# ecmwf/anemoi-core

Hardware: AMD Instinct MI355X
Metric: forward nodes*channels/sec on O96 GraphTransformer (higher is better)
Workload: dtype bf16; 1 GPU; AnemoiModelEncProcDec forward, O96 data grid (40320 nodes, 84 vars x 2 steps) -> icosphere res 5 hidden mesh (10242 nodes, 81840 edges), GraphTransformer processor 16 layers x 512 ch x 16 heads, enc 62912 / dec 120960 edges, batch 1; parallelism=single GPU, hip_graph=True, graph_equals_eager=True, graph_segments=1

## Files before the change

### anemoi_core_amd/_lib.py

```python
from __future__ import annotations

import ctypes as C
import os
import threading

ABI_VERSION = 13
LIB_PATH = os.path.join(os.path.dirname(os.path.abspath(__file__)), "lib", "libanemoi_hip.so")

F32, BF16, F16 = 0, 1, 2
ACT_NONE, ACT_GELU = 0, 1
E_INVALID, E_UNSUPPORTED, E_LAUNCH = -1, -2, -3

_p, _i64, _i32, _f = C.c_void_p, C.c_int64, C.c_int32, C.c_float

SIGNATURES = {
    "anemoi_hip_abi_version": ([], C.c_int),
    "anemoi_hip_last_error": ([], C.c_char_p),
    "anemoi_gt_attention_fwd": ([_p, _i64, _p, _i64, _p, _i64, _p, _i64, _p, _p, _p, _i64, _p, _i64, _p, _i32, _i32, _i32, _i32, C.c_int, _p], C.c_int),
    "anemoi_gt_attention_bwd": ([_p, _i64, _p, _i64, _p, _i64, _p, _i64, _p, _i64, _p, _p, _i64, _p, _p, _p, _p, _p,
                                 _p, _i64, _p, _i64, _p, _i64, _p, _i64, _p, _p, _i32, _i32, _i32, _i32, _i32, C.c_int, _p], C.c_int),
    "anemoi_gt_attention_dropout_fwd": ([_p, _i64, _p, _i64, _p, _i64, _p, _i64, _p, _p, _p, _i64, _p, _i64, _p, _i32, _i32, _i32, _i32, _f, C.c_uint64,
                                         C.c_int, _p], C.c_int),
    "anemoi_gt_attention_dropout_bwd": ([_p, _i64, _p, _i64, _p, _i64, _p, _i64, _p, _i64, _p, _p, _i64, _p, _p, _p, _p, _p,
                                         _p, _i64, _p, _i64, _p, _i64, _p, _i64, _p, _p, _i32, _i32, _i32, _i32, _i32, _f, C.c_uint64, C.c_int, _p], C.c_int),
    "anemoi_attention_dropout_mask": ([_p, _i32, _i32, _f, C.c_uint64, _p], C.c_int),
    "anemoi_gt_attention_fused_edge_fwd": ([_p, _i64, _p, _i64, _p, _i64, _p, _i32, _p, _p, _p, _p, _p, _i64, _p, _i64, _p, _i32, _i32, _i32, _i32, C.c_int, _p], C.c_int),
    "anemoi_pack_edge_weights": ([_p, _p, _p, _i32, _i32, _i32, C.c_int, _p], C.c_int),
    "anemoi_pack_edge_features": ([_p, _i64, _p, _i32, _i32, _i32, C.c_int, _p], C.c_int),
    "anemoi_reduce_workspace_bytes": ([_i32], _i64),
    "anemoi_layernorm_bwd": ([_p, _i64, _p, _p, _i64, _p, _i64, _p, _p, _p, _i32, _i32, _f, C.c_int, _p], C.c_int),
    "anemoi_colsum": ([_p, _i64, _p, _p, _i32, _i32, C.c_int, _p], C.c_int),
    "anemoi_gelu_fwd": ([_p, _i64, _p, _i64, _i32, _i32, C.c_int, _p], C.c_int),
    "anemoi_gelu_bwd": ([_p, _i64, _p, _i64, _p, _i64, _i32, _i32, C.c_int, _p], C.c_int),
    "anemoi_cond_layernorm_bwd": ([_p, _i64, _p, _i64, _p, _i64, _p, _i64, _p, _i64, _i32, _i32, _f, C.c_int, _p], C.c_int),
    "anemoi_cond_layernorm_fwd": ([_p, _i64, _p, _i64, _p, _i64, _p, _i64, _i32, _i32, _f, C.c_int, _p], C.c_int),
    "anemoi_assemble_input": ([_p, _i64, _i64, _i32, _i32, _p, _i64, _i32, _p, _i64, _i32, _i32, C.c_int, _p], C.c_int),
    "anemoi_assemble_output": ([_p, _i64, _p, _i64, _p, _p, _i64, _i32, _i32, C.c_int, _p], C.c_int),
    "anemoi_assemble_input_norm": ([_p, C.c_int, _i64, _i64, _i32, _i32, _p, _p, _p, _i64, _i32, _p, _i64, _i32, _i32, C.c_int, _p], C.c_int),
    "anemoi_assemble_output_norm": ([_p, _i64, C.c_int, _p, _i64, _p, _p, _p, _p, _i64, _i32, _i32, C.c_int, _p], C.c_int),
    "anemoi_affine_columns": ([_p, _i64, _p, _i64, _p, _p, _i32, _i32, _i32, C.c_int, _p], C.c_int),
    "anemoi_bound_columns": ([_p, _i64, _i32, _i32, _p, _p, _i32, C.c_int, _p], C.c_int),
    "anemoi_layernorm_fwd": ([_p, _i64, _p, _p, _p, _i64, _p, _i64, _i32, _i32, _f, C.c_int, _p], C.c_int),
    "anemoi_gt_attention_fused_edge_bwd_partial_floats": ([_i32, _i32, _i32], _i64),
    "anemoi_gt_attention_fused_edge_bwd": ([_p, _i64, _p, _i64, _p, _i64, _p, _i32, _p, _p, _i64, _p, _p, _i64, _p, _p, _p, _p, _p,
                                            _p, _i64, _p, _i64, _p, _i64, _p, _p, _p, _p, _p, _p, _p, _p, _i64, _p, _i64,
                                            _i32, _i32, _i32, _i32, _i32, C.c_int, _p], C.c_int),
    "anemoi_linear_wgrad_workspace_bytes": ([_i32, _i32, _i32], _i64),
    "anemoi_linear_wgrad": ([_p, _i64, _p, _i64, _p, _i64, _p, _p, _i32, _i32, _i32, C.c_int, _p], C.c_int),
    "anemoi_linear_splitk_f32": ([_p, _i64, _p, _i64, _p, _i64, _i32, _i32, _i32, _i32, C.c_int, _p], C.c_int),
    "anemoi_linear_stats_fwd": ([_p, _i64, _i32, _p, _i64, _p, _p, _i64, _p, _i64, _p, _i32, _i32, C.c_int, _p], C.c_int),
    "anemoi_linear_lnfold_fwd": ([_p, _i64, _i32, _p, _i64, _p, _p, _p, _i32, _f, C.c_int, _p, _i64, _i32, _i32, C.c_int, _p], C.c_int),
    "anemoi_linear_fwd": ([_p, _i64, _i32, _p, _i64, _i32, _p, _i64, _p, _p, _i64, _p, _p, _i64, _p, _p, _i64, _p, _i64, _i32, _i32, C.c_int, C.c_int, _p], C.c_int),
    "anemoi_linear_fwd_pre": ([_p, _i64, _i32, _p, _i64, _i32, _p, _i64, _p, _p, _i64, _p, _p, _i64, _p, _p, _i64, _p, _i64, _p, _i64, _i32, _i32,
                               C.c_int, C.c_int, _p], C.c_int),
    "anemoi_edge_ln_residual_segment_sum_fwd": ([_p, _i64, _p, _i64, _p, _p, _f, _p, _p, _i64, _p, _i64, _i32, _i32, C.c_int, _p], C.c_int),
    "anemoi_segment_sum_rows": ([_p, _i64, _p, _p, _p, _i64, _i32, _i32, C.c_int, _p], C.c_int),
    "anemoi_gather_add_rows": ([_p, _i64, _p, _i64, _p, _p, _i64, _i32, _i32, C.c_int, _p], C.c_int),
    "anemoi_transpose_pad": ([_p, _i64, _p, _i64, _i32, _i32, _i32, C.c_int, _p], C.c_int),
    "anemoi_glu_fwd": ([_p, _i64, _p, _i64, _i32, _i32, _i32, C.c_int, _p], C.c_int),
    "anemoi_glu_bwd": ([_p, _i64, _p, _i64, _p, _i64, _i32, _i32, _i32, C.c_int, _p], C.c_int),
    "anemoi_gather_rows": ([_p, _i64, _p, _p, _i64, _i32, _i32, C.c_int, _p], C.c_int),
    "anemoi_peer_alloc": ([C.POINTER(_p), _i64, _i32], C.c_int),
    "anemoi_peer_free": ([_p], C.c_int),
    "anemoi_peer_export": ([_p, _p], C.c_int),
    "anemoi_peer_open": ([_p, C.POINTER(_p)], C.c_int),
    "anemoi_peer_close": ([_p], C.c_int),
    "anemoi_gt_chain_rows_per_tile": ([_i32], C.c_int),
    "anemoi_gt_chain2_fwd": ([_p, C.c_int, _p], C.c_int),
    "anemoi_gt_rowchain_fwd": ([_p, C.c_int, _p], C.c_int),
    "anemoi_gt_cluster_chain_fwd": ([_p, C.c_int, _p], C.c_int),
    "anemoi_gt_cluster_chain_workspace_bytes": ([], _i64),
    "anemoi_gnn_edge_chain_fwd": ([_p, _i64, _p, _i64, _p, _p, _i64, _p, _p, _p, _p, _p, _p, _p, _p, _p, _f, _p, _i64, _i32, _i32, C.c_int, _p], C.c_int),
    "anemoi_gnn_mlp_chain_fwd": ([_p, _i64, _i32, _p, _p, _p, _p, _p, _p, _p, _p, _f, _p, _i64, _p, _i64, _i32, _i32, C.c_int, _p], C.c_int),
    "anemoi_gnn_node_chain_segsum_fwd": ([_p, _i64, _p, _i64, _p, _p, _p, _p, _p, _p, _p, _p, _p, _f, _p, _i64, _p, _p, _i32, _p, _i64, _i32, _i32,
                                          C.c_int, _p], C.c_int),
    "anemoi_gnn_node_chain_fwd": ([_p, _i64, _p, _i64, _p, _p, _p, _p, _p, _p, _p, _p, _f, _p, _i64, _p, _p, _i32, _p, _i64, _i32, _i32, C.c_int, _p], C.c_int),
    "anemoi_peer_exchange_rows": ([_p, _i64, _p, _p, _i32, _i32, _i32, _p, _p, _i64, _p], C.c_int),
}


EXPERIMENT_SIGNATURES = {
    "anemoi_gt_chain_fwd": ([_p, C.c_int, _p], C.c_int),
    "anemoi_gnn_edge_chain_timeline": ([_p, _i64, _p, _i64, _p, _p, _i64, _p, _p, _p, _p, _p, _p, _p, _p, _p, _f, _p, _i64, _i32, _p, _p], C.c_int),
}


class HipLibraryError(RuntimeError):
    pass


_lock = threading.Lock()
_lib = None


def load(path: str | None = None):
    global _lib
    if _lib is not None:
        return _lib
    with _lock:
        if _lib is not None:
            return _lib
        path = path or os.environ.get("ANEMOI_HIP_LIB", LIB_PATH)
        if not os.path.exists(path):
            raise HipLibraryError(
                f"{path} not found: build it with `python -m anemoi_core_amd.build` (hipcc, gfx950). "
                "anemoi_core_amd has no CPU / eager fallback."
            )
        try:
            lib = C.CDLL(path)
        except OSError as e:
            raise HipLibraryError(f"cannot load {path}: {e}") from e
        for name, (argtypes, restype) in SIGNATURES.items():
            try:
                fn = getattr(lib, name)
            except AttributeError as e:
                raise HipLibraryError(f"{path} does not export {name}; rebuild the library") from e
            fn.argtypes = argtypes
            fn.restype = restype
        for name, (argtypes, restype) in EXPERIMENT_SIGNATURES.items():
            fn = getattr(lib, name, None)
            if fn is not None:
# ... 18 lines not shown
```

### anemoi_core_amd/build.py

```python
from __future__ import annotations

import os
import shutil
import subprocess
import sys
from concurrent.futures import ThreadPoolExecutor

PKG = os.path.dirname(os.path.abspath(__file__))
REPO = os.path.dirname(PKG)
CSRC = os.path.join(PKG, "csrc")
LIBDIR = os.path.join(PKG, "lib")
LIBPATH = os.path.join(LIBDIR, "libanemoi_hip.so")
EXT_PATH = os.path.join(LIBDIR, "libanemoi_torch.so")
INCLUDE = os.path.join(REPO, "include")

SOURCES = ["lib.cpp", "gt_attention.hip", "gt_attention_bwd.hip", "rowwise.hip", "rowwise_bwd.hip", "linear.hip", "wgrad.hip", "peer.hip", "gt_chain2.hip", "gt_rowchain.hip", "gt_cluster_chain.hip", "gnn_chain.hip"]
EXPERIMENT_SOURCES = ["experiments/gt_chain.hip", "experiments/gnn_chain2.hip"]
EXP_LIBPATH = os.path.join(LIBDIR, "libanemoi_hip_exp.so")
ARCH = "gfx950"


def _hipcc() -> str:
    for cand in (os.environ.get("HIPCC"), shutil.which("hipcc"), "/opt/rocm/bin/hipcc"):
        if cand and os.path.exists(cand):
            return cand
    raise RuntimeError("hipcc not found (need ROCm >= 7.0)")


def _newer(target: str, deps: list[str]) -> bool:
    if not os.path.exists(target):
        return False
    t = os.path.getmtime(target)
    return all(os.path.getmtime(d) <= t for d in deps)


def _deps(path: str, dirs: list[str], seen: set | None = None) -> list[str]:
    import re

    seen = set() if seen is None else seen
    if path in seen:
        return []
    seen.add(path)
    out = [path]
    for inc in re.findall(r'^\s*#include\s+"([^"]+)"', open(path).read(), flags=re.M):
        for d in [os.path.dirname(path), *dirs]:
            cand = os.path.join(d, inc)
            if os.path.exists(cand):
                out += _deps(cand, dirs, seen)
                break
    return out


def build_library(force: bool = False, verbose: bool = True, extra_flags: tuple[str, ...] = (), experiments: bool = False) -> str:
    os.makedirs(LIBDIR, exist_ok=True)
    objdir = os.path.join(LIBDIR, "obj_exp" if experiments else "obj")
    os.makedirs(objdir, exist_ok=True)
    hipcc = _hipcc()
    headers = [os.path.join(CSRC, "common.h"), os.path.join(CSRC, "chain_core.h"), os.path.join(CSRC, "chain2_core.h"), os.path.join(CSRC, "gnn_chain_args.h"), os.path.join(INCLUDE, "anemoi_hip.h")]
    flags = ["-O3", "-std=c++17", "-fPIC", f"--offload-arch={ARCH}", "-I", INCLUDE, "-I", CSRC, "-Wall", "-Wno-unused-function", *extra_flags]
    sources, libpath = SOURCES, LIBPATH
    inc_dirs = [CSRC, INCLUDE] + ([os.path.join(CSRC, "experiments")] if experiments else [])
    if experiments:
        flags += ["-DANEMOI_EXPERIMENTS", "-I", os.path.join(CSRC, "experiments")]
        headers.append(os.path.join(CSRC, "experiments", "anemoi_hip_experiments.h"))
        sources, libpath = SOURCES + EXPERIMENT_SOURCES, EXP_LIBPATH

    def compile_one(src: str) -> str:
        path = os.path.join(CSRC, src)
        obj = os.path.join(objdir, os.path.splitext(os.path.basename(src))[0] + ".o")
        if not force and _newer(obj, _deps(path, inc_dirs)):
            return obj
        cmd = [hipcc, *flags, "-x", "hip", "-c", path, "-o", obj]
        if verbose:
            print("[build]", " ".join(cmd), flush=True)
        subprocess.run(cmd, check=True)
        return obj

    with ThreadPoolExecutor(max_workers=min(4, len(sources))) as ex:
        objs = list(ex.map(compile_one, sources))
    if force or not _newer(libpath, objs):
        cmd = [hipcc, "-shared", "-fPIC", f"--offload-arch={ARCH}", "-o", libpath, *objs]
        if verbose:
            print("[build]", " ".join(cmd), flush=True)
        subprocess.run(cmd, check=True)
    if not experiments:
        build_torch_extension(hipcc, force=force, verbose=verbose)
    return libpath


def build_torch_extension(hipcc: str, force: bool = False, verbose: bool = True) -> str:
    import torch

    src = os.path.join(CSRC, "torch_binding.cpp")
    stamp = EXT_PATH + ".torch_version"
    stamped = open(stamp).read().strip() if os.path.exists(stamp) else None
    if not force and stamped in (None, torch.__version__) and _newer(EXT_PATH, [src, os.path.join(INCLUDE, "anemoi_hip.h"), LIBPATH]):
        if stamped is None:
            open(stamp, "w").write(torch.__version__)
        return EXT_PATH
    troot = os.path.dirname(torch.__file__)
    rocm = os.environ.get("ROCM_PATH", "/opt/rocm")
    cmd = [hipcc, "-O2", "-std=c++17", "-fPIC", "-shared", "-D__HIP_PLATFORM_AMD__=1", "-DUSE_ROCM=1",
           f"-D_GLIBCXX_USE_CXX11_ABI={int(torch._C._GLIBCXX_USE_CXX11_ABI)}", "-I", INCLUDE, "-I", os.path.join(troot, "include"),
           "-I", os.path.join(troot, "include", "torch", "csrc", "api", "include"), "-I", os.path.join(rocm, "include"), src, "-o", EXT_PATH,
           "-L", LIBDIR, "-lanemoi_hip", "-L", os.path.join(troot, "lib"), "-lc10", "-lc10_hip", "-ltorch_cpu", "-ltorch", "-ltorch_hip",
           "-Wl,-rpath,$ORIGIN"]
    if verbose:
        print("[build]", " ".join(cmd), flush=True)
    subprocess.run(cmd, check=True)
    open(stamp, "w").write(torch.__version__)
    return EXT_PATH
# ... 5 lines not shown
```

### anemoi_core_amd/csrc/gt_chain2.hip

```cpp
#include "chain2_core.h"

namespace anemoi {

struct Chain2Args {
  const void* attn;  int64_t ld_attn;
  const void* xres;  int64_t ld_x;
  const char* wp;
  const char* w1;    int hc;
  const char* w2;
  const char* wq;    int qc;
  int qn;
  int q_cols;
  const void* vec;
  float eps1, epsq;
  const void* extra; int64_t ld_extra;
  void* xout;        int64_t ld_out;
  void* qout;        int64_t ld_q;
  int n_rows, rows_per_tile, n_tiles;
  int prio_a;
  int prio_q;
  int dbg;
  int warm;
  int b_delay;
  unsigned long long* timeline;
};
constexpr int kTl2Slots = 48;
constexpr int kRed2Off = 3 * kBufBytes;
constexpr int kVecOff = kRed2Off + kPanel * 4 * 2 * 4;
constexpr int kVecMaxElems = 6144;
constexpr int kChain2Smem = kVecOff + kVecMaxElems * 2;
constexpr int kVecMaxElemsTl = 5120;
constexpr int kTl2Off = kVecOff + kVecMaxElemsTl * 2;
static_assert(kChain2Smem <= 160 * 1024 && kTl2Off + 8 * kTl2Slots * 8 <= 160 * 1024, "LDS budget");

struct Ctx2 {
  int lane, wq, wave;
  uint32_t loff;
  int tl_n;
};
template <bool TL>
__device__ __forceinline__ void stamp2(Ctx2& c, unsigned char* smem) {
  if constexpr (TL) {
    if (c.tl_n < kTl2Slots) {
      const unsigned long long now = __builtin_readcyclecounter();
      if (c.lane == 0) reinterpret_cast<unsigned long long*>(smem + kTl2Off)[c.wave * kTl2Slots + c.tl_n] = now;
    }
    ++c.tl_n;
  }
}
struct VecCopy {
  u32x4 v[2];
  __device__ __forceinline__ void request(const Chain2Args& a, int tid) {
    const int n16 = (1024 + 512 * a.hc + a.q_cols) / 8;
// ... 264 lines not shown
  if (c.wave < 4) {
    if (kExperiments && a.prio_a == 2) __builtin_amdgcn_s_setprio(2);
    role_a<T, TL, PART>(a, c, smem);
  } else {
    role_b<T, TL>(a, c, smem);
  }
  if constexpr (TL) {
    asm volatile("s_waitcnt lgkmcnt(0)" ::: "memory");
    if (c.lane < kTl2Slots)
      a.timeline[((size_t)blockIdx.x * 8 + c.wave) * kTl2Slots + c.lane] =
          c.lane < c.tl_n ? reinterpret_cast<const unsigned long long*>(smem + kTl2Off)[c.wave * kTl2Slots + c.lane] : 0ull;
  }
}

template <typename T>
static int launch_chain2(const Chain2Args& a, hipStream_t st) {
  static PerDeviceOnce attr_once;
  attr_once.run([&] {
    (void)hipFuncSetAttribute(reinterpret_cast<const void*>(&gt_chain2_kernel<T>), hipFuncAttributeMaxDynamicSharedMemorySize, kChain2Smem);
    (void)hipFuncSetAttribute(reinterpret_cast<const void*>(&gt_chain2_kernel<T, false, true>), hipFuncAttributeMaxDynamicSharedMemorySize, kChain2Smem);
  });
  static const int even_grid = ANEMOI_EXPERIMENT_ENV("ANEMOI_CHAIN2_EVEN_GRID", 1, 0, 1);
  int grid = a.n_tiles < 256 ? a.n_tiles : 256;
  static const int max_grid = ANEMOI_EXPERIMENT_ENV("ANEMOI_CHAIN2_MAX_GRID", 256, 8, 256);
  if (even_grid && a.n_tiles > 256) {
    const int rounds = (a.n_tiles + max_grid - 1) / max_grid;
    grid = (a.n_tiles + rounds - 1) / rounds;
  }
#ifdef ANEMOI_EXPERIMENTS
  if (a.timeline != nullptr) {
    static PerDeviceOnce tl_once;
    tl_once.run([&] {
      (void)hipFuncSetAttribute(reinterpret_cast<const void*>(&gt_chain2_kernel<T, true>), hipFuncAttributeMaxDynamicSharedMemorySize, kTl2Off + 8 * kTl2Slots * 8);
      (void)hipFuncSetAttribute(reinterpret_cast<const void*>(&gt_chain2_kernel<T, true, true>), hipFuncAttributeMaxDynamicSharedMemorySize, kTl2Off + 8 * kTl2Slots * 8);
    });
    if (grid < 256) hipLaunchKernelGGL((gt_chain2_kernel<T, true, true>), dim3(grid), dim3(512), kTl2Off + 8 * kTl2Slots * 8, st, a);
    else hipLaunchKernelGGL((gt_chain2_kernel<T, true>), dim3(grid), dim3(512), kTl2Off + 8 * kTl2Slots * 8, st, a);
    return check_launch("gt_chain2_kernel<timeline>");
  }
#endif
  if (grid < 256) hipLaunchKernelGGL((gt_chain2_kernel<T, false, true>), dim3(grid), dim3(512), kChain2Smem, st, a);
  else hipLaunchKernelGGL((gt_chain2_kernel<T>), dim3(grid), dim3(512), kChain2Smem, st, a);
  return check_launch("gt_chain2_kernel");
}

}

using namespace anemoi;

extern "C" int anemoi_gt_chain_rows_per_tile(int32_t n_rows) {
  static const int forced = env_int(getenv("ANEMOI_CHAIN_ROWS"), 0, 0, kPanel);
  (void)n_rows;
  return forced > 0 ? forced : kPanel;
}

extern "C" int anemoi_gt_chain2_fwd(const anemoi_gt_chain2_args_t* p, anemoi_dtype_t dtype, void* stream) {
  ANEMOI_REQUIRE(p != nullptr, "gt_chain2_fwd: null argument block");
  ANEMOI_REQUIRE(dtype == ANEMOI_BF16 || dtype == ANEMOI_F16, "gt_chain2_fwd: 16-bit model dtypes only");
  ANEMOI_REQUIRE(p->n_rows >= 0 && p->channels == kCh, "gt_chain2_fwd: channels=%d (this kernel is built for %d)", p->channels, kCh);
  if (p->n_rows == 0) return ANEMOI_OK;
  const bool narrow = p->q_out_features > 0 && p->q_out_features < kCh;
  ANEMOI_REQUIRE(p->hidden > 0 && p->hidden % kCh == 0 && p->q_out_features >= 0 && (narrow ? p->q_out_features % 128 == 0 : p->q_out_features % kCh == 0),
                 "gt_chain2_fwd: hidden=%d must be a multiple of %d, q_out_features=%d a multiple of %d (or 128, 256, 384)", p->hidden, kCh, p->q_out_features, kCh);
  const int n_vec = 2 * kCh + p->hidden + p->q_out_features;
  if (n_vec > (p->timeline != nullptr ? kVecMaxElemsTl : kVecMaxElems)) return ANEMOI_E_UNSUPPORTED;
  ANEMOI_REQUIRE(p->attn && p->x_res && p->wp && p->w1 && p->w2 && p->vec && (p->x_out || p->q_out_features > 0), "gt_chain2_fwd: null operand");
  ANEMOI_REQUIRE(p->q_out_features == 0 || (p->wq && p->q_out), "gt_chain2_fwd: the trailing projection needs wq and q_out");
  ANEMOI_REQUIRE(p->extra == nullptr || p->x_out != nullptr, "gt_chain2_fwd: a second residual needs x_out");
  const auto al16 = [](const void* q) { return (reinterpret_cast<uintptr_t>(q) & 15) == 0; };
  ANEMOI_REQUIRE(al16(p->attn) && al16(p->x_res) && al16(p->wp) && al16(p->w1) && al16(p->w2) && al16(p->x_out) && al16(p->wq) && al16(p->q_out) &&
                     al16(p->extra) && al16(p->vec),
                 "gt_chain2_fwd: operands must be 16-byte aligned");
  ANEMOI_REQUIRE(p->ld_attn >= kCh && p->ld_x >= kCh && (p->x_out == nullptr || (p->ld_out >= kCh && p->ld_out % 8 == 0)) && p->ld_attn % 8 == 0 && p->ld_x % 8 == 0 &&
                     (p->extra == nullptr || (p->ld_extra >= kCh && p->ld_extra % 8 == 0)) &&
                     (p->q_out_features == 0 || (p->ld_q >= p->q_out_features && p->ld_q % 8 == 0)),
                 "gt_chain2_fwd: leading dimensions too small or not multiples of 8 elements (rows move as 16-byte pieces)");
  Chain2Args a{};
  a.attn = p->attn; a.ld_attn = p->ld_attn;
  a.xres = p->x_res; a.ld_x = p->ld_x;
  a.wp = (const char*)p->wp;
  a.w1 = (const char*)p->w1; a.hc = p->hidden / kCh;
  a.w2 = (const char*)p->w2;
  a.wq = (const char*)p->wq; a.qc = narrow ? 1 : p->q_out_features / kCh;
  a.qn = narrow ? p->q_out_features / 128 : 0; a.q_cols = p->q_out_features;
  a.vec = p->vec;
  a.eps1 = p->ln1_eps; a.epsq = p->lnq_eps;
  a.extra = p->extra; a.ld_extra = p->ld_extra;
  a.xout = p->x_out; a.ld_out = p->ld_out;
  a.qout = p->q_out; a.ld_q = p->ld_q;
  if (!kExperiments && p->timeline != nullptr) {
    set_error("gt_chain2_fwd: the in-kernel timeline is part of the experiments build only (python -m anemoi_core_amd.build --experiments)");
    return ANEMOI_E_UNSUPPORTED;
  }
  a.timeline = reinterpret_cast<unsigned long long*>(p->timeline);
  static const int prio_a = ANEMOI_EXPERIMENT_ENV("ANEMOI_CHAIN2_PRIO_A", 0, 0, 2);
  a.prio_a = prio_a;
  static const int dbg = ANEMOI_EXPERIMENT_ENV("ANEMOI_CHAIN2_DBG", 0, 0, 15);
  a.dbg = dbg;
  static const int prio_q = ANEMOI_EXPERIMENT_ENV("ANEMOI_CHAIN2_PRIO_Q", 0, 0, 1);
  a.prio_q = prio_q;
  static const int warm = ANEMOI_EXPERIMENT_ENV("ANEMOI_CHAIN2_WARM", 1, 0, 1);
  a.warm = warm;
  static const int b_delay = ANEMOI_EXPERIMENT_ENV("ANEMOI_CHAIN2_B_DELAY", 0, 0, 40);
  a.b_delay = b_delay;
  a.n_rows = p->n_rows;
  a.rows_per_tile = p->rows_per_tile > 0 ? p->rows_per_tile : anemoi_gt_chain_rows_per_tile(p->n_rows);
  ANEMOI_REQUIRE(a.rows_per_tile <= kPanel, "gt_chain2_fwd: rows_per_tile=%d exceeds the %d-row panel", a.rows_per_tile, kPanel);
  a.n_tiles = (a.n_rows + a.rows_per_tile - 1) / a.rows_per_tile;
  hipStream_t st = as_stream(stream);
  return dtype == ANEMOI_BF16 ? launch_chain2<bf16_t>(a, st) : launch_chain2<f16_t>(a, st);
}
```

### include/anemoi_hip.h

```cpp
#ifndef ANEMOI_HIP_H
#define ANEMOI_HIP_H

#include <stdint.h>

#ifdef __cplusplus
extern "C" {
#endif

#define ANEMOI_HIP_ABI_VERSION 13

typedef enum { ANEMOI_F32 = 0, ANEMOI_BF16 = 1, ANEMOI_F16 = 2 } anemoi_dtype_t;
typedef enum { ANEMOI_ACT_NONE = 0, ANEMOI_ACT_GELU = 1 } anemoi_act_t;

#define ANEMOI_OK 0
#define ANEMOI_E_INVALID (-1)
#define ANEMOI_E_UNSUPPORTED (-2)
#define ANEMOI_E_LAUNCH (-3)

int anemoi_hip_abi_version(void);
const char* anemoi_hip_last_error(void);

int anemoi_gt_attention_fwd(const void* q, int64_t ldq, const void* k, int64_t ldk, const void* v, int64_t ldv,
                            const void* e, int64_t lde, const int32_t* row, const int32_t* colptr,
                            const void* addend, int64_t ldadd, void* out, int64_t ldo, float* lse,
                            int32_t n_dst, int32_t n_src, int32_t H, int32_t C, anemoi_dtype_t dtype, void* stream);

int anemoi_gt_attention_bwd(const void* q, int64_t ldq, const void* k, int64_t ldk, const void* v, int64_t ldv,
                            const void* e, int64_t lde, const void* out, int64_t ldo, const float* lse,
                            const void* d_out, int64_t lddo, const int32_t* row, const int32_t* colptr,
                            const int32_t* rowptr, const int32_t* edge_ids, const int32_t* edge_dst,
                            void* dq, int64_t lddq, void* dk, int64_t lddk, void* dv, int64_t lddv, void* de, int64_t ldde,
                            float* p_ws, float* ds_ws, int32_t n_dst, int32_t n_src, int32_t n_edges, int32_t H, int32_t C,
                            anemoi_dtype_t dtype, void* stream);

int anemoi_gt_attention_dropout_fwd(const void* q, int64_t ldq, const void* k, int64_t ldk, const void* v, int64_t ldv,
                                    const void* e, int64_t lde, const int32_t* row, const int32_t* colptr,
                                    const void* addend, int64_t ldadd, void* out, int64_t ldo, float* lse,
                                    int32_t n_dst, int32_t n_src, int32_t H, int32_t C, float drop_p, uint64_t drop_seed,
                                    anemoi_dtype_t dtype, void* stream);
int anemoi_gt_attention_dropout_bwd(const void* q, int64_t ldq, const void* k, int64_t ldk, const void* v, int64_t ldv,
                                    const void* e, int64_t lde, const void* out, int64_t ldo, const float* lse,
                                    const void* d_out, int64_t lddo, const int32_t* row, const int32_t* colptr,
                                    const int32_t* rowptr, const int32_t* edge_ids, const int32_t* edge_dst,
                                    void* dq, int64_t lddq, void* dk, int64_t lddk, void* dv, int64_t lddv, void* de, int64_t ldde,
                                    float* p_ws, float* ds_ws, int32_t n_dst, int32_t n_src, int32_t n_edges, int32_t H, int32_t C,
                                    float drop_p, uint64_t drop_seed, anemoi_dtype_t dtype, void* stream);
int anemoi_attention_dropout_mask(float* out, int32_t n_edges, int32_t H, float drop_p, uint64_t drop_seed, void* stream);

int anemoi_gt_attention_fused_edge_fwd(const void* q, int64_t ldq, const void* k, int64_t ldk, const void* v, int64_t ldv,
                                       const float* edge_feat, int32_t fe_pad, const float* w_packed,
                                       const int32_t* row, const int32_t* colptr, const int32_t* dst_order, const void* addend, int64_t ldadd,
                                       void* out, int64_t ldo, float* lse, int32_t n_dst, int32_t n_src, int32_t H,
                                       int32_t C, anemoi_dtype_t dtype, void* stream);

int64_t anemoi_gt_attention_fused_edge_bwd_partial_floats(int32_t H, int32_t C, int32_t fe_pad);
int anemoi_gt_attention_fused_edge_bwd(const void* q, int64_t ldq, const void* k, int64_t ldk, const void* v, int64_t ldv,
                                       const float* edge_feat, int32_t fe_pad, const float* w_packed, const void* out, int64_t ldo,
                                       const float* lse, const void* d_out, int64_t lddo, const int32_t* row, const int32_t* colptr,
                                       const int32_t* rowptr, const int32_t* edge_ids, const int32_t* edge_dst, void* dq,
                                       int64_t lddq, void* dk, int64_t lddk, void* dv, int64_t lddv, float* d_w_packed,
                                       float* d_edge_feat, float* p_ws, float* ds_ws, float* sf_ws, float* qg_ws, float* part_ws,
                                       const void* addend, int64_t ldadd, void* d_addend, int64_t lddadd, int32_t n_dst,
// ... 77 lines not shown
                           int32_t n_out, int32_t D, anemoi_dtype_t dtype, void* stream);

int anemoi_transpose_pad(const void* x, int64_t ldx, void* out, int64_t ldo, int32_t n_rows, int32_t n_cols, int32_t n_pad,
                         anemoi_dtype_t dtype, void* stream);

int anemoi_glu_fwd(const void* gate_value, int64_t ldgv, void* out, int64_t ldo, int32_t n_rows, int32_t D, int32_t kind,
                   anemoi_dtype_t dtype, void* stream);
int anemoi_glu_bwd(const void* gate_value, int64_t ldgv, const void* d_out, int64_t lddo, void* d_gate_value, int64_t lddgv,
                   int32_t n_rows, int32_t D, int32_t kind, anemoi_dtype_t dtype, void* stream);


int anemoi_assemble_input_norm(const void* x, anemoi_dtype_t x_dtype, int64_t ld_t, int64_t ldx, int32_t T_steps, int32_t V,
                               const float* col_mul, const float* col_add, const void* attrs, int64_t lda, int32_t A, void* out,
                               int64_t ldo, int32_t W, int32_t n_rows, anemoi_dtype_t dtype, void* stream);

int anemoi_assemble_output_norm(const void* x_out, int64_t ldx, anemoi_dtype_t model_dtype, const void* x_skip, int64_t lds,
                                const int32_t* col_map, const float* col_mul, const float* col_add, void* out, int64_t ldo,
                                int32_t n_rows, int32_t n_cols, anemoi_dtype_t dtype, void* stream);

int anemoi_affine_columns(const void* x, int64_t ldx, void* y, int64_t ldy, const float* col_mul, const float* col_add,
                          int32_t inverse, int32_t n_rows, int32_t V, anemoi_dtype_t dtype, void* stream);

#define ANEMOI_PEER_MEM_DEFAULT 0
#define ANEMOI_PEER_MEM_FINEGRAINED 1
#define ANEMOI_PEER_MEM_UNCACHED 2
#define ANEMOI_PEER_HANDLE_BYTES 64
int anemoi_peer_alloc(void** ptr, int64_t bytes, int32_t kind);
int anemoi_peer_free(void* ptr);
int anemoi_peer_export(void* ptr, void* handle_out );
int anemoi_peer_open(const void* handle , void** ptr_out);
int anemoi_peer_close(void* ptr);

int anemoi_peer_exchange_rows(const void* src, int64_t ld_src_bytes, const int32_t* send_index, const int64_t* table,
                              int32_t n_peers, int32_t row_bytes, int32_t total_rows, uint32_t* local_flags, uint32_t* status,
                              int64_t timeout_ticks, void* stream);

typedef struct anemoi_gt_chain2_args {
  const void* attn;   int64_t ld_attn;
  const void* x_res;  int64_t ld_x;
  const void* wp;
  const void* w1;     int32_t hidden;
  const void* w2;
  const void* wq;     int32_t q_out_features;
  const void* vec;
  float ln1_eps;      float lnq_eps;
  const void* extra;  int64_t ld_extra;
  void* x_out;        int64_t ld_out;
  void* q_out;        int64_t ld_q;
  int32_t n_rows;     int32_t channels;   int32_t rows_per_tile;
  void* timeline;
} anemoi_gt_chain2_args_t;
int anemoi_gt_chain2_fwd(const anemoi_gt_chain2_args_t* args, anemoi_dtype_t dtype, void* stream);
int anemoi_gt_chain_rows_per_tile(int32_t n_rows);

typedef struct anemoi_gt_rowchain_args {
  const void* x;      int64_t ld_x;       int32_t in_features;
  const void* we;
  const void* wq;     int32_t q_out_features;
  const void* vec;
  float ln_eps;
  void* x_out;        int64_t ld_out;
  void* q_out;        int64_t ld_q;
  int32_t n_rows;     int32_t channels;   int32_t rows_per_tile;
} anemoi_gt_rowchain_args_t;
int anemoi_gt_rowchain_fwd(const anemoi_gt_rowchain_args_t* args, anemoi_dtype_t dtype, void* stream);

typedef struct anemoi_gt_cluster_chain_args {
  const void* attn;   int64_t ld_attn;
  const void* x_res;  int64_t ld_x;
  const void* wp;
  const void* w1;     int32_t hidden;
  const void* w2;
  const void* wq;     int32_t q_out_features;
  const void* vec;
  float ln1_eps;      float lnq_eps;
  const void* extra;  int64_t ld_extra;
  void* x_out;        int64_t ld_out;
  void* q_out;        int64_t ld_q;
  void* ln_out;       int64_t ld_ln;
  void* q_out2;       int64_t ld_q2;      int32_t q_split;
  void* workspace;    int64_t workspace_bytes;
  int32_t n_rows;     int32_t channels;
} anemoi_gt_cluster_chain_args_t;
int anemoi_gt_cluster_chain_fwd(const anemoi_gt_cluster_chain_args_t* args, anemoi_dtype_t dtype, void* stream);
int64_t anemoi_gt_cluster_chain_workspace_bytes(void);

int anemoi_gnn_edge_chain_fwd(const void* e, int64_t ld_e, const void* g1, int64_t ld_g1, const int32_t* idx1, const void* g2, int64_t ld_g2,
                              const int32_t* idx2, const void* w0, const void* b0, const void* w1, const void* b1, const void* w2, const void* b2,
                              const void* ln_w, const void* ln_b, float eps, void* e_new, int64_t ld_o, int32_t n_rows, int32_t channels,
                              anemoi_dtype_t dtype, void* stream);
int anemoi_gnn_mlp_chain_fwd(const void* x, int64_t ld_x, int32_t in_features, const void* w0, const void* b0, const void* w1, const void* b1,
                             const void* w2, const void* b2, const void* ln_w, const void* ln_b, float eps, const void* res, int64_t ld_res,
                             void* out, int64_t ld_o, int32_t n_rows, int32_t channels, anemoi_dtype_t dtype, void* stream);

int anemoi_gnn_node_chain_fwd(const void* x, int64_t ld_x, const void* agg, int64_t ld_a, const void* wa, const void* ba, const void* wb,
                              const void* bb, const void* wc, const void* bc, const void* ln_w, const void* ln_b, float eps, void* x_out,
                              int64_t ld_o, const void* wt, const void* bt, int32_t t_out_features, void* t_out, int64_t ld_t, int32_t n_rows,
                              int32_t channels, anemoi_dtype_t dtype, void* stream);
int anemoi_gnn_node_chain_segsum_fwd(const void* x, int64_t ld_x, const void* edge_rows, int64_t ld_e, const int32_t* seg_ptr, const void* wa,
                                     const void* ba, const void* wb, const void* bb, const void* wc, const void* bc, const void* ln_w,
                                     const void* ln_b, float eps, void* x_out, int64_t ld_o, const void* wt, const void* bt,
                                     int32_t t_out_features, void* t_out, int64_t ld_t, int32_t n_rows, int32_t channels,
                                     anemoi_dtype_t dtype, void* stream);


#ifdef __cplusplus
// ... 4 lines not shown
```

Baseline: 8.889 billion nodes*channels/s.

## Add a 96-row panel variant of the chain2 fused MLP kernel for large row counts

Adds a second fused projection/LayerNorm/MLP/q-projection kernel that processes 96-row tiles instead of the default panel. Each weight fragment streamed from global memory is reused across twice as many rows, cutting weight traffic per row. A planner picks this form when the tile count exceeds 256 (or when forced by env) and sizes a balanced persistent grid. The cost is more accumulator registers and LDS per block, which limits occupancy, and the 96-row kernel does not support the timeline path.

```diff
diff --git a/anemoi_core_amd/_lib.py b/anemoi_core_amd/_lib.py
--- a/anemoi_core_amd/_lib.py
+++ b/anemoi_core_amd/_lib.py
@@ -4,7 +4,7 @@
 import os
 import threading
 
-ABI_VERSION = 13
+ABI_VERSION = 14
 LIB_PATH = os.path.join(os.path.dirname(os.path.abspath(__file__)), "lib", "libanemoi_hip.so")
 
 F32, BF16, F16 = 0, 1, 2
@@ -67,6 +67,7 @@
     "anemoi_peer_close": ([_p], C.c_int),
     "anemoi_gt_chain_rows_per_tile": ([_i32], C.c_int),
     "anemoi_gt_chain2_fwd": ([_p, C.c_int, _p], C.c_int),
+    "anemoi_gt_chain2_plan": ([_i32, _i32, _i32, _i32, _p, _p], C.c_int),
     "anemoi_gt_rowchain_fwd": ([_p, C.c_int, _p], C.c_int),
     "anemoi_gt_cluster_chain_fwd": ([_p, C.c_int, _p], C.c_int),
     "anemoi_gt_cluster_chain_workspace_bytes": ([], _i64),
diff --git a/anemoi_core_amd/build.py b/anemoi_core_amd/build.py
--- a/anemoi_core_amd/build.py
+++ b/anemoi_core_amd/build.py
@@ -14,7 +14,7 @@
 EXT_PATH = os.path.join(LIBDIR, "libanemoi_torch.so")
 INCLUDE = os.path.join(REPO, "include")
 
-SOURCES = ["lib.cpp", "gt_attention.hip", "gt_attention_bwd.hip", "rowwise.hip", "rowwise_bwd.hip", "linear.hip", "wgrad.hip", "peer.hip", "gt_chain2.hip", "gt_rowchain.hip", "gt_cluster_chain.hip", "gnn_chain.hip"]
+SOURCES = ["lib.cpp", "gt_attention.hip", "gt_attention_bwd.hip", "rowwise.hip", "rowwise_bwd.hip", "linear.hip", "wgrad.hip", "peer.hip", "gt_chain2.hip", "gt_chain2_p96.hip", "gt_rowchain.hip", "gt_cluster_chain.hip", "gnn_chain.hip"]
 EXPERIMENT_SOURCES = ["experiments/gt_chain.hip", "experiments/gnn_chain2.hip"]
 EXP_LIBPATH = os.path.join(LIBDIR, "libanemoi_hip_exp.so")
 ARCH = "gfx950"
@@ -56,7 +56,7 @@
     objdir = os.path.join(LIBDIR, "obj_exp" if experiments else "obj")
     os.makedirs(objdir, exist_ok=True)
     hipcc = _hipcc()
-    headers = [os.path.join(CSRC, "common.h"), os.path.join(CSRC, "chain_core.h"), os.path.join(CSRC, "chain2_core.h"), os.path.join(CSRC, "gnn_chain_args.h"), os.path.join(INCLUDE, "anemoi_hip.h")]
+    headers = [os.path.join(CSRC, "common.h"), os.path.join(CSRC, "chain_core.h"), os.path.join(CSRC, "chain2_core.h"), os.path.join(CSRC, "chain2_p96.h"), os.path.join(CSRC, "gnn_chain_args.h"), os.path.join(INCLUDE, "anemoi_hip.h")]
     flags = ["-O3", "-std=c++17", "-fPIC", f"--offload-arch={ARCH}", "-I", INCLUDE, "-I", CSRC, "-Wall", "-Wno-unused-function", *extra_flags]
     sources, libpath = SOURCES, LIBPATH
     inc_dirs = [CSRC, INCLUDE] + ([os.path.join(CSRC, "experiments")] if experiments else [])
diff --git a/anemoi_core_amd/csrc/chain2_p96.h b/anemoi_core_amd/csrc/chain2_p96.h
--- /dev/null
+++ b/anemoi_core_amd/csrc/chain2_p96.h
@@ -0,0 +1,26 @@
+#pragma once
+#include "common.h"
+
+namespace anemoi {
+
+struct Chain2P96Args {
+  const void* attn;  int64_t ld_attn;
+  const void* xres;  int64_t ld_x;
+  const char* wp;
+  const char* w1;    int hc;
+  const char* w2;
+  const char* wq;    int qc;
+  int q_cols;
+  const void* vec;
+  float eps1, epsq;
+  const void* extra; int64_t ld_extra;
+  void* xout;        int64_t ld_out;
+  void* qout;        int64_t ld_q;
+  int n_rows, rows_per_tile, n_tiles;
+};
+constexpr int kP96Rows = 96;
+constexpr int kP96VecMaxElems = 5120;
+
+int launch_chain2_p96(const Chain2P96Args& a, bool bf16, int grid, hipStream_t st);
+
+}
diff --git a/anemoi_core_amd/csrc/gt_chain2.hip b/anemoi_core_amd/csrc/gt_chain2.hip
--- a/anemoi_core_amd/csrc/gt_chain2.hip
+++ b/anemoi_core_amd/csrc/gt_chain2.hip
@@ -1,4 +1,7 @@
 #include "chain2_core.h"
+#include "chain2_p96.h"
+
+#include <cstring>
 
 namespace anemoi {
 
@@ -369,6 +372,35 @@
   static const int forced = env_int(getenv("ANEMOI_CHAIN_ROWS"), 0, 0, kPanel);
   (void)n_rows;
   return forced > 0 ? forced : kPanel;
+}
+
+struct Chain2Plan {
+  int form;
+  int rows, tiles, grid;
+};
+static Chain2Plan chain2_plan(int n_rows, int hidden, int q_out, int forced, int panel, bool timeline) {
+  const bool fits96 = !timeline && hidden > 0 && hidden % kCh == 0 && 2 * kCh + hidden + q_out <= kP96VecMaxElems;
+  Chain2Plan p{};
+  if (forced > kPanel) p.form = 1;
+  else if (forced > 0 || panel == 48 || !fits96) p.form = 0;
+  else if (panel == 96) p.form = 1;
+  else p.form = (n_rows + kPanel - 1) / kPanel > 256 ? 1 : 0;
+  p.rows = forced > 0 ? forced : (p.form ? kP96Rows : kPanel);
+  p.tiles = n_rows > 0 ? (n_rows + p.rows - 1) / p.rows : 0;
+  p.grid = p.tiles < 256 ? p.tiles : (p.tiles + (p.tiles + 255) / 256 - 1) / ((p.tiles + 255) / 256);
+  return p;
+}
+static int chain2_panel_switch(const char* e) {
+  const int v = (e == nullptr || strcmp(e, "auto") == 0) ? 0 : env_int(e, 0, 48, 96);
+  return v == 48 || v == 96 ? v : 0;
+}
+
+extern "C" int anemoi_gt_chain2_plan(int32_t n_rows, int32_t hidden, int32_t q_out_features, int32_t rows_per_tile, int32_t* panel_rows, int32_t* grid) {
+  if (rows_per_tile < 0 || rows_per_tile > kP96Rows || n_rows < 0) return -1;
+  const Chain2Plan p = chain2_plan(n_rows, hidden, q_out_features, rows_per_tile, chain2_panel_switch(getenv("ANEMOI_CHAIN2_PANEL")), false);
+  if (panel_rows != nullptr) *panel_rows = p.rows;
+  if (grid != nullptr) *grid = p.grid;
+  return p.form;
 }
 
 extern "C" int anemoi_gt_chain2_fwd(const anemoi_gt_chain2_args_t* p, anemoi_dtype_t dtype, void* stream) {
@@ -421,9 +453,28 @@
   static const int b_delay = ANEMOI_EXPERIMENT_ENV("ANEMOI_CHAIN2_B_DELAY", 0, 0, 40);
   a.b_delay = b_delay;
   a.n_rows = p->n_rows;
-  a.rows_per_tile = p->rows_per_tile > 0 ? p->rows_per_tile : anemoi_gt_chain_rows_per_tile(p->n_rows);
-  ANEMOI_REQUIRE(a.rows_per_tile <= kPanel, "gt_chain2_fwd: rows_per_tile=%d exceeds the %d-row panel", a.rows_per_tile, kPanel);
-  a.n_tiles = (a.n_rows + a.rows_per_tile - 1) / a.rows_per_tile;
+  ANEMOI_REQUIRE(p->rows_per_tile >= 0 && p->rows_per_tile <= kP96Rows, "gt_chain2_fwd: rows_per_tile=%d exceeds the %d-row panel", p->rows_per_tile, kP96Rows);
+  static const int forced_env = env_int(getenv("ANEMOI_CHAIN_ROWS"), 0, 0, kPanel);
+  static const int panel = chain2_panel_switch(getenv("ANEMOI_CHAIN2_PANEL"));
+  const int forced = p->rows_per_tile > 0 ? p->rows_per_tile : forced_env;
+  const Chain2Plan plan = chain2_plan(p->n_rows, p->hidden, p->q_out_features, forced, panel, p->timeline != nullptr);
   hipStream_t st = as_stream(stream);
+  if (plan.form == 1) {
+    ANEMOI_REQUIRE(2 * kCh + p->hidden + p->q_out_features <= kP96VecMaxElems && p->timeline == nullptr,
+                   "gt_chain2_fwd: rows_per_tile=%d needs the 96-row kernel, which holds at most %d vector entries and has no timeline", forced, kP96VecMaxElems);
+    Chain2P96Args b{};
+    b.attn = a.attn; b.ld_attn = a.ld_attn;
+    b.xres = a.xres; b.ld_x = a.ld_x;
+    b.wp = a.wp; b.w1 = a.w1; b.hc = a.hc; b.w2 = a.w2;
+    b.wq = a.wq; b.qc = a.qc; b.q_cols = a.q_cols;
+    b.vec = a.vec; b.eps1 = a.eps1; b.epsq = a.epsq;
+    b.extra = a.extra; b.ld_extra = a.ld_extra;
+    b.xout = a.xout; b.ld_out = a.ld_out;
+    b.qout = a.qout; b.ld_q = a.ld_q;
+    b.n_rows = a.n_rows; b.rows_per_tile = plan.rows; b.n_tiles = plan.tiles;
+    return launch_chain2_p96(b, dtype == ANEMOI_BF16, plan.grid, st);
+  }
+  a.rows_per_tile = plan.rows;
+  a.n_tiles = plan.tiles;
   return dtype == ANEMOI_BF16 ? launch_chain2<bf16_t>(a, st) : launch_chain2<f16_t>(a, st);
 }
diff --git a/anemoi_core_amd/csrc/gt_chain2_p96.hip b/anemoi_core_amd/csrc/gt_chain2_p96.hip
--- /dev/null
+++ b/anemoi_core_amd/csrc/gt_chain2_p96.hip
@@ -0,0 +1,381 @@
+#include "chain2_core.h"
+#include "chain2_p96.h"
+
+namespace anemoi {
+
+constexpr int kP96HRow = 512;
+constexpr int kP96R = 0;
+constexpr int kP96H = kP96R + kP96Rows * kRowBytes;
+constexpr int kP96Red = kP96H + kP96Rows * kP96HRow;
+constexpr int kP96Vec = kP96Red + kP96Rows * 8 * 2 * 4;
+constexpr int kP96Smem = kP96Vec + kP96VecMaxElems * 2;
+static_assert(kP96Smem <= 160 * 1024, "LDS budget");
+static_assert(kP96Rows * kP96HRow == 48 * kRowBytes, "H holds a [48][512] staging half");
+
+template <typename T, int F, int RB>
+__device__ __forceinline__ void gemm96(const unsigned char* abuf, int lane, frag8 (&ring)[8], const char* cur, const char* nxt, bool nxt_half,
+                                       uint32_t loff, f32x4 (&acc)[6][F], int ng) {
+  static_assert(F == 2 || F == 4, "fragments per K-step");
+  constexpr int G = 8 / F;
+  asm volatile("" : "+v"(lane));
+  const int x = lane & 15, ks = lane >> 4;
+  const unsigned char* arow = abuf + x * RB;
+  frag8 fa[6];
+#pragma unroll
+  for (int mi = 0; mi < 6; ++mi) fa[mi] = *reinterpret_cast<const frag8*>(arow + mi * 16 * RB + ((ks ^ x) << 4));
+  const int last = ng * G - 1;
+#pragma unroll 1
+  for (int q = 0; q < ng; ++q) {
+    const bool tail = q == ng - 1;
+    const gptr_t gb = uniform_ptr(tail ? nxt : cur + (q + 1) * (G * 4096));
+#pragma unroll
+    for (int j = 0; j < G; ++j) {
+      const int st = q * G + j;
+      const int sn = st < last ? st + 1 : last;
+      frag8 fn[6];
+      if constexpr (F == 4) {
+#pragma unroll
+        for (int mi = 0; mi < 6; ++mi) fn[mi] = *reinterpret_cast<const frag8*>(arow + mi * 16 * RB + (((sn * 4 + ks) ^ x) << 4));
+      }
+      __builtin_amdgcn_sched_barrier(0);
+#pragma unroll
+      for (int ni = 0; ni < F; ++ni) {
+        const int s = j * F + ni;
+#pragma unroll
+        for (int mi = 0; mi < 6; ++mi) acc[mi][ni] = cmfma<T>(ring[s], fa[mi], acc[mi][ni]);
+        const uint32_t offn = nxt_half ? (s / 2) * 4096 + (s % 2) * 1024 : (s / 4) * 4096 + (s % 4) * 1024;
+        const uint32_t off = tail ? offn : (s / F) * 4096 + (s % F) * 1024;
+        ring[s] = *reinterpret_cast<gfrag_t>(gb + (loff + off));
+        __builtin_amdgcn_sched_barrier(0);
+      }
+      if constexpr (F == 4) {
+#pragma unroll
+        for (int mi = 0; mi < 6; ++mi) fa[mi] = fn[mi];
+      } else {
+#pragma unroll
+        for (int mi = 0; mi < 6; ++mi) fa[mi] = *reinterpret_cast<const frag8*>(arow + mi * 16 * RB + (((sn * 4 + ks) ^ x) << 4));
+      }
+      __builtin_amdgcn_sched_barrier(0);
+    }
+  }
+}
+__device__ __forceinline__ void ring_prologue96(frag8 (&ring)[8], const char* f0, uint32_t loff) {
+#pragma unroll
+  for (int s = 0; s < 8; ++s) {
+    ring[s] = *reinterpret_cast<gfrag_t>(uniform_ptr(f0 + (s / 4) * 4096 + (s % 4) * 1024) + loff);
+    __builtin_amdgcn_sched_barrier(0);
+  }
+}
+
+template <typename T, int F, bool ADD>
+__device__ __forceinline__ void bias96(f32x4 (&acc)[6][F], const unsigned char* vec, int col0, int lane) {
+  asm volatile("" : "+v"(lane));
+  const int g = lane >> 4;
+#pragma unroll
+  for (int ni = 0; ni < F; ++ni) {
+    float b[4];
+    unpack4<T>(*reinterpret_cast<const u32x2*>(vec + (col0 + ni * 16 + g * 4) * 2), b);
+#pragma unroll
+    for (int mi = 0; mi < 6; ++mi)
+      acc[mi][ni] = ADD ? f32x4{acc[mi][ni][0] + b[0], acc[mi][ni][1] + b[1], acc[mi][ni][2] + b[2], acc[mi][ni][3] + b[3]} : f32x4{b[0], b[1], b[2], b[3]};
+  }
+}
+
+__device__ __forceinline__ void stats_band(const f32x4 (&a)[4], float* red, int row, int g, int w) {
+  float s = 0.f;
+#pragma unroll
+  for (int ni = 0; ni < 4; ++ni) s += (a[ni][0] + a[ni][1]) + (a[ni][2] + a[ni][3]);
+  s += __shfl_xor(s, 16, 64);
+  s += __shfl_xor(s, 32, 64);
+  const float mw = s * (1.0f / 64.0f);
+  float q = 0.f;
+#pragma unroll
+  for (int ni = 0; ni < 4; ++ni)
+#pragma unroll
+    for (int r = 0; r < 4; ++r) {
+      const float d = a[ni][r] - mw;
+      q = fmaf(d, d, q);
+    }
+  q += __shfl_xor(q, 16, 64);
+  q += __shfl_xor(q, 32, 64);
+  if (g == 0) *reinterpret_cast<float2*>(red + (row * 8 + w) * 2) = make_float2(mw, q);
+}
+
+template <typename T>
+__device__ __forceinline__ void x1_rows(f32x4 (&acc)[6][4], const unsigned char* rows, const unsigned char* vec, float* red, int lane, int w) {
+  const LaneCtx lc = lane_ctx(lane, w);
+#pragma unroll
+  for (int mi = 0; mi < 6; ++mi) {
+    const unsigned char* rrow = rows + (mi * 16 + lc.x) * kRowBytes;
+    u32x2 rb[4], rr[4];
+#pragma unroll
+    for (int ni = 0; ni < 4; ++ni) {
+      rb[ni] = *reinterpret_cast<const u32x2*>(vec + (w * 64 + ni * 16 + lc.g * 4) * 2);
+      rr[ni] = *reinterpret_cast<const u32x2*>(rrow + lc.coff[ni]);
+    }
+    __builtin_amdgcn_sched_barrier(0);
+#pragma unroll
+    for (int ni = 0; ni < 4; ++ni) {
+      float o[4] = {acc[mi][ni][0], acc[mi][ni][1], acc[mi][ni][2], acc[mi][ni][3]};
+      float b[4], r[4];
+      unpack4<T>(rb[ni], b);
+      unpack4<T>(rr[ni], r);
+#pragma unroll
+      for (int k = 0; k < 4; ++k) o[k] += b[k] + r[k];
+      unpack4<T>(pack4<T>(o), o);
+      acc[mi][ni] = f32x4{o[0], o[1], o[2], o[3]};
+    }
+    stats_band(acc[mi], red, mi * 16 + lc.x, lc.g, w);
+  }
+}
+
+template <typename T>
+__device__ __forceinline__ void normalise96(const f32x4 (&acc)[6][4], const float* red, float eps, unsigned char* dst, int lane, int w) {
+  const LaneCtx lc = lane_ctx(lane, w);
+#pragma unroll
+  for (int mi = 0; mi < 6; ++mi) {
+    const f32x4* pr = reinterpret_cast<const f32x4*>(red + (mi * 16 + lc.x) * 16);
+    const f32x4 p0 = pr[0], p1 = pr[1], p2 = pr[2], p3 = pr[3];
+    const float mu = (((p0[0] + p0[2]) + (p1[0] + p1[2])) + ((p2[0] + p2[2]) + (p3[0] + p3[2]))) * 0.125f;
+    float m2 = ((p0[1] + p0[3]) + (p1[1] + p1[3])) + ((p2[1] + p2[3]) + (p3[1] + p3[3]));
+    const float d0 = p0[0] - mu, d1 = p0[2] - mu, d2 = p1[0] - mu, d3 = p1[2] - mu;
+    const float d4 = p2[0] - mu, d5 = p2[2] - mu, d6 = p3[0] - mu, d7 = p3[2] - mu;
+    m2 = fmaf(64.0f, ((d0 * d0 + d1 * d1) + (d2 * d2 + d3 * d3)) + ((d4 * d4 + d5 * d5) + (d6 * d6 + d7 * d7)), m2);
+    const float rstd = rsqrtf(m2 * (1.0f / (float)kCh) + eps);
+    const float nm = -mu * rstd;
+    unsigned char* drow = dst + (mi * 16 + lc.x) * kRowBytes;
+#pragma unroll
+    for (int ni = 0; ni < 4; ++ni) {
+      float o[4];
+#pragma unroll
+      for (int r = 0; r < 4; ++r) o[r] = fmaf(acc[mi][ni][r], rstd, nm);
+      *reinterpret_cast<u32x2*>(drow + lc.coff[ni]) = pack4<T>(o);
+    }
+  }
+}
+
+template <typename T>
+__device__ __forceinline__ void gelu96(const f32x4 (&acc)[6][2], unsigned char* hb, int lane, int w) {
+  asm volatile("" : "+v"(lane));
+  const int x = lane & 15, g = lane >> 4;
+#pragma unroll
+  for (int mi = 0; mi < 6; ++mi) {
+    unsigned char* drow = hb + (mi * 16 + x) * kP96HRow;
+#pragma unroll
+    for (int ni = 0; ni < 2; ++ni) {
+      float o[4] = {acc[mi][ni][0], acc[mi][ni][1], acc[mi][ni][2], acc[mi][ni][3]};
+      gelu_fast2(o[0], o[1]);
+      gelu_fast2(o[2], o[3]);
+      *reinterpret_cast<u32x2*>(drow + ((((w * 4 + ni * 2 + (g >> 1)) ^ x) << 4) + (g & 1) * 8)) = pack4<T>(o);
+      __builtin_amdgcn_sched_barrier(0);
+    }
+  }
+}
+
+template <typename T, bool EXTRA, bool BACK>
+__device__ __forceinline__ void store_half(f32x4 (&acc)[6][4], int h, unsigned char* hb, T* out, int64_t ld, const T* extra, int64_t ld_extra,
+                                           int row0, int nr, int lane, int w) {
+  {
+    const LaneCtx lc = lane_ctx(lane, w);
+#pragma unroll
+    for (int i = 0; i < 3; ++i) {
+      unsigned char* drow = hb + (i * 16 + lc.x) * kRowBytes;
+#pragma unroll
+      for (int ni = 0; ni < 4; ++ni) {
+        float o[4] = {acc[3 * h + i][ni][0], acc[3 * h + i][ni][1], acc[3 * h + i][ni][2], acc[3 * h + i][ni][3]};
+        const u32x2 pk = pack4<T>(o);
+        *reinterpret_cast<u32x2*>(drow + lc.coff[ni]) = pk;
+        unpack4<T>(pk, o);
+        acc[3 * h + i][ni] = f32x4{o[0], o[1], o[2], o[3]};
+      }
+    }
+  }
+  asm volatile("s_waitcnt lgkmcnt(0)" ::: "memory");
+  int l0 = lane;
+  asm volatile("" : "+v"(l0));
+  const int rl = l0 >> 3, sl = l0 & 7;
+#pragma unroll
+  for (int it = 0; it < 6; ++it) {
+    const int row = it * 8 + rl;
+    const int prow = 48 * h + row;
+    unsigned char* slot = hb + row * kRowBytes + (((w * 8 + sl) ^ (row & 15)) << 4);
+    u32x4 v = *reinterpret_cast<const u32x4*>(slot);
+    if (prow < nr) {
+      if constexpr (EXTRA) {
+        const u32x4 e = *reinterpret_cast<const u32x4*>(extra + (int64_t)(row0 + prow) * ld_extra + w * 64 + sl * 8);
+        float p[4], s[4];
+        unpack4<T>(u32x2{v[0], v[1]}, p);
+        unpack4<T>(u32x2{e[0], e[1]}, s);
+#pragma unroll
+        for (int r = 0; r < 4; ++r) p[r] += s[r];
+        const u32x2 lo = pack4<T>(p);
+        unpack4<T>(u32x2{v[2], v[3]}, p);
+        unpack4<T>(u32x2{e[2], e[3]}, s);
+#pragma unroll
+        for (int r = 0; r < 4; ++r) p[r] += s[r];
+        const u32x2 hi = pack4<T>(p);
+        v = u32x4{lo[0], lo[1], hi[0], hi[1]};
+        if constexpr (BACK) *reinterpret_cast<u32x4*>(slot) = v;
+      }
+      if (out != nullptr) stream_store(v, reinterpret_cast<u32x4*>(out + (int64_t)(row0 + prow) * ld + w * 64 + sl * 8));
+    }
+  }
+  if constexpr (BACK) {
+    asm volatile("s_waitcnt lgkmcnt(0)" ::: "memory");
+    const LaneCtx lc = lane_ctx(lane, w);
+#pragma unroll
+    for (int i = 0; i < 3; ++i)
+#pragma unroll
+      for (int ni = 0; ni < 4; ++ni) {
+        float o[4];
+        unpack4<T>(*reinterpret_cast<const u32x2*>(hb + (i * 16 + lc.x) * kRowBytes + lc.coff[ni]), o);
+        acc[3 * h + i][ni] = f32x4{o[0], o[1], o[2], o[3]};
+      }
+  }
+}
+
+template <typename T>
+__global__ __launch_bounds__(512, 1) void gt_chain2_kernel_p96(Chain2P96Args a) {
+  extern __shared__ __attribute__((aligned(16))) unsigned char smem[];
+  const int tid = threadIdx.x;
+  const int lane = tid & 63;
+  const int w = __builtin_amdgcn_readfirstlane(tid >> 6);
+  const uint32_t loff = lane * 16;
+  if ((int)blockIdx.x >= a.n_tiles) return;
+  unsigned char* const R = smem + kP96R;
+  unsigned char* const H = smem + kP96H;
+  float* const red = reinterpret_cast<float*>(smem + kP96Red);
+  unsigned char* const vec = smem + kP96Vec;
+  const int hc = a.hc, nch = 2 * hc, qc = a.qc;
+  const int64_t s2 = (int64_t)hc * kSlab;
+  const char* const wpw = a.wp + (int64_t)w * kSlab;
+  auto w1c = [&](int c) { return a.w1 + (int64_t)(4 * c + (w >> 1)) * kSlab + (w & 1) * 2048; };
+  auto w2c = [&](int c) { return a.w2 + (int64_t)w * s2 + (int64_t)c * 32768; };
+  auto qact = [&](int k) { return k < qc && k * 512 + w * 64 < a.q_cols; };
+  auto wqc = [&](int k) { return a.wq + (int64_t)(8 * k + w) * kSlab; };
+  const char* const after_mlp = qact(0) ? wqc(0) : wpw;
+  frag8 ring[8];
+  f32x4 acc[6][4];
+  Warm warm;
+  warm_init<true>(warm, w & 1, lane);
+  auto touch = [&](const char* sa, int64_t pa, const char* sb, int64_t pb) {
+    touch_done<true>(warm);
+    if (w < 2) { if (sa != nullptr) touch_share<true>(warm, sa, pa, w & 1, lane); }
+    else if (w < 4 && sb != nullptr) touch_share<true>(warm, sb, pb, w & 1, lane);
+  };
+  {
+    const int r0 = (int)blockIdx.x * a.rows_per_tile;
+    u32x4 v[2];
+    const int n16 = (1024 + 512 * hc + a.q_cols) / 8;
+    load_rows12<T>((const T*)a.attn, a.ld_attn, r0, min(a.rows_per_tile, a.n_rows - r0), R, lane, w, [&] {
+#pragma unroll
+      for (int k = 0; k < 2; ++k) v[k] = reinterpret_cast<const u32x4*>(a.vec)[min(tid + 512 * k, n16 - 1)];
+      ring_prologue96(ring, wpw, loff);
+      if (w < 2) touch_share<true>(warm, a.wp, kSlab, w & 1, lane);
+    });
+#pragma unroll
+    for (int k = 0; k < 2; ++k)
+      if (tid + 512 * k < n16) reinterpret_cast<u32x4*>(vec)[tid + 512 * k] = v[k];
+    lds_barrier();
+  }
+  for (int tile = blockIdx.x;;) {
+    const int r0 = tile * a.rows_per_tile;
+    const int nr = min(a.rows_per_tile, a.n_rows - r0);
+#pragma unroll
+    for (int mi = 0; mi < 6; ++mi)
+#pragma unroll
+      for (int ni = 0; ni < 4; ++ni) acc[mi][ni] = f32x4{0.f, 0.f, 0.f, 0.f};
+    gemm96<T, 4, kRowBytes>(R, lane, ring, wpw, w1c(0), true, loff, acc, 8);
+    touch(a.w1, kSlab, a.w2, s2);
+    lds_barrier();
+    load_rows12<T>((const T*)a.xres, a.ld_x, r0, nr, R, lane, w, [] {});
+    lds_barrier();
+    x1_rows<T>(acc, R, vec, red, lane, w);
+    lds_barrier();
+    normalise96<T>(acc, red, a.eps1, R, lane, w);
+    bias96<T, 4, true>(acc, vec, 512 + 512 * hc + w * 64, lane);
+    lds_barrier();
+    for (int c = 0; c < nch; ++c) {
+      {
+        f32x4 acc1[6][2];
+        bias96<T, 2, false>(acc1, vec, 512 + 256 * c + w * 32, lane);
+        gemm96<T, 2, kRowBytes>(R, lane, ring, w1c(c), w2c(c), false, loff, acc1, 4);
+        if ((c & 1) == 0) {
+          const int k = (c >> 1) + 1;
+          if (k < hc) touch(a.w1 + (int64_t)(8 * k) * kSlab, kSlab, a.w2 + (int64_t)k * kSlab, s2);
+          else touch(qc > 0 && a.q_cols >= 512 ? a.wq : nullptr, kSlab, qc > 1 ? a.wq + (int64_t)8 * kSlab : nullptr, kSlab);
+        }
+        gelu96<T>(acc1, H, lane, w);
+      }
+      lds_barrier();
+      gemm96<T, 4, kP96HRow>(H, lane, ring, w2c(c), c + 1 < nch ? w1c(c + 1) : after_mlp, c + 1 < nch, loff, acc, 4);
+      lds_barrier();
+    }
+    const T* const extra = (const T*)a.extra;
+    T* const xout = (T*)a.xout;
+    if (extra != nullptr) {
+      if (qc > 0) {
+        store_half<T, true, true>(acc, 0, H, xout, a.ld_out, extra, a.ld_extra, r0, nr, lane, w);
+        store_half<T, true, true>(acc, 1, H, xout, a.ld_out, extra, a.ld_extra, r0, nr, lane, w);
+      } else {
+        store_half<T, true, false>(acc, 0, H, xout, a.ld_out, extra, a.ld_extra, r0, nr, lane, w);
+        store_half<T, true, false>(acc, 1, H, xout, a.ld_out, extra, a.ld_extra, r0, nr, lane, w);
+      }
+    } else if (xout != nullptr) {
+      store_half<T, false, false>(acc, 0, H, xout, a.ld_out, nullptr, 0, r0, nr, lane, w);
+      store_half<T, false, false>(acc, 1, H, xout, a.ld_out, nullptr, 0, r0, nr, lane, w);
+    } else {
+#pragma unroll
+      for (int mi = 0; mi < 6; ++mi)
+#pragma unroll
+        for (int ni = 0; ni < 4; ++ni) {
+          float o[4] = {acc[mi][ni][0], acc[mi][ni][1], acc[mi][ni][2], acc[mi][ni][3]};
+          unpack4<T>(pack4<T>(o), o);
+          acc[mi][ni] = f32x4{o[0], o[1], o[2], o[3]};
+        }
+    }
+    if (qc > 0) {
+      {
+        int l0 = lane;
+        asm volatile("" : "+v"(l0));
+#pragma unroll
+        for (int mi = 0; mi < 6; ++mi) stats_band(acc[mi], red, mi * 16 + (l0 & 15), l0 >> 4, w);
+      }
+      lds_barrier();
+      normalise96<T>(acc, red, a.epsq, R, lane, w);
+      lds_barrier();
+      for (int k = 0; k < qc; ++k) {
+        if (!qact(k)) break;
+        bias96<T, 4, false>(acc, vec, 1024 + 512 * hc + 512 * k + w * 64, lane);
+        gemm96<T, 4, kRowBytes>(R, lane, ring, wqc(k), qact(k + 1) ? wqc(k + 1) : wpw, false, loff, acc, 8);
+        touch(qact(k + 2) ? a.wq + (int64_t)(8 * (k + 2)) * kSlab : nullptr, kSlab, nullptr, 0);
+        T* const qo = (T*)a.qout + 512 * k;
+        store_half<T, false, false>(acc, 0, H, qo, a.ld_q, nullptr, 0, r0, nr, lane, w);
+        store_half<T, false, false>(acc, 1, H, qo, a.ld_q, nullptr, 0, r0, nr, lane, w);
+      }
+      lds_barrier();
+    }
+    tile += (int)gridDim.x;
+    if (tile >= a.n_tiles) break;
+    const int rn = tile * a.rows_per_tile;
+    load_rows12<T>((const T*)a.attn, a.ld_attn, rn, min(a.rows_per_tile, a.n_rows - rn), R, lane, w, [] {});
+    lds_barrier();
+  }
+  touch_done<true>(warm);
+}
+
+template <typename T>
+static int launch_p96(const Chain2P96Args& a, int grid, hipStream_t st) {
+  static PerDeviceOnce attr_once;
+  attr_once.run([&] {
+    (void)hipFuncSetAttribute(reinterpret_cast<const void*>(&gt_chain2_kernel_p96<T>), hipFuncAttributeMaxDynamicSharedMemorySize, kP96Smem);
+  });
+  hipLaunchKernelGGL((gt_chain2_kernel_p96<T>), dim3(grid), dim3(512), kP96Smem, st, a);
+  return check_launch("gt_chain2_kernel_p96");
+}
+
+int launch_chain2_p96(const Chain2P96Args& a, bool bf16, int grid, hipStream_t st) {
+  return bf16 ? launch_p96<bf16_t>(a, grid, st) : launch_p96<f16_t>(a, grid, st);
+}
+
+}
diff --git a/include/anemoi_hip.h b/include/anemoi_hip.h
--- a/include/anemoi_hip.h
+++ b/include/anemoi_hip.h
@@ -7,7 +7,7 @@
 extern "C" {
 #endif
 
-#define ANEMOI_HIP_ABI_VERSION 13
+#define ANEMOI_HIP_ABI_VERSION 14
 
 typedef enum { ANEMOI_F32 = 0, ANEMOI_BF16 = 1, ANEMOI_F16 = 2 } anemoi_dtype_t;
 typedef enum { ANEMOI_ACT_NONE = 0, ANEMOI_ACT_GELU = 1 } anemoi_act_t;
@@ -191,6 +191,7 @@
 } anemoi_gt_chain2_args_t;
 int anemoi_gt_chain2_fwd(const anemoi_gt_chain2_args_t* args, anemoi_dtype_t dtype, void* stream);
 int anemoi_gt_chain_rows_per_tile(int32_t n_rows);
+int anemoi_gt_chain2_plan(int32_t n_rows, int32_t hidden, int32_t q_out_features, int32_t rows_per_tile, int32_t* panel_rows, int32_t* grid);
 
 typedef struct anemoi_gt_rowchain_args {
   const void* x;      int64_t ld_x;       int32_t in_features;
```

Result: faster. 9.007 billion nodes*channels/s (median of 6 runs) (+1.3%).
